# laboshinl/loam_velodyne

Hardware: AMD Instinct MI355X
Metric: sweeps/sec (64-ring, 1M-pt map): feature extraction + odometry + scan-to-map registration (higher is better)
Workload: dtype f32

## Files before the change

### loam_velodyne_amd/csrc/dev_math.hpp

```cpp
#pragma once
#include <hip/hip_runtime.h>
#include <cfloat>

namespace loamx {

struct Pose {
  float rx, ry, rz, tx, ty, tz;
  float srx, crx, sry, cry, srz, crz;
};

__host__ __device__ inline void pose_set_angles(Pose& p, float rx, float ry, float rz) {
  p.rx = rx; p.ry = ry; p.rz = rz;
  p.srx = (float)sin((double)rx); p.crx = (float)cos((double)rx);
  p.sry = (float)sin((double)ry); p.cry = (float)cos((double)ry);
  p.srz = (float)sin((double)rz); p.crz = (float)cos((double)rz);
}

__host__ __device__ inline void rot_x(float& y, float& z, float c, float s) {
  float y0 = y;
  y = c * y0 - s * z;
  z = s * y0 + c * z;
}
__host__ __device__ inline void rot_y(float& x, float& z, float c, float s) {
  float x0 = x;
// ... 332 lines not shown
__device__ __forceinline__ bool degeneracy_projector(const float* AtA, float thr, float* P, float* ws) {
  if (certainly_not_degenerate(AtA, thr)) return false;
  return degeneracy_projector_full(AtA, thr, P, ws);
}
__device__ __forceinline__ bool degeneracy_projector_full(const float* AtA, float thr, float* P, float* ws) {
  float w[6];
  float* V = ws + 72;
  float* V2 = ws + 108;
  float* Vi = ws + 144;
  eig6_sym(AtA, w, V, ws);
  for (int k = 0; k < 36; k++) V2[k] = V[k];
  bool degenerate = false;
  {
    bool go = true;
#pragma unroll
    for (int i = 0; i < 6; i++) {
      if (go && w[i] < thr) {
        for (int j = 0; j < 6; j++) V2[i * 6 + j] = 0.f;
        degenerate = true;
      } else {
        go = false;
      }
    }
  }
  if (!inverse6(V, Vi, ws)) {
    for (int k = 0; k < 36; k++) P[k] = (k % 7 == 0) ? 1.f : 0.f;
    return degenerate;
  }
  for (int r = 0; r < 6; r++)
    for (int c = 0; c < 6; c++) {
      float s = 0.f;
      for (int k = 0; k < 6; k++) s += Vi[r * 6 + k] * V2[k * 6 + c];
      P[r * 6 + c] = s;
    }
  return degenerate;
}

__device__ __forceinline__ float lane_get(float x, int lane) { return __int_as_float(__builtin_amdgcn_readlane(__float_as_int(x), lane)); }

__device__ __forceinline__ float qr_solve6_lanes(const float* AtA, const float* AtB) {
  const int gl = (int)(threadIdx.x & 63);
  float a[6];
#pragma unroll
  for (int r = 0; r < 6; r++) a[r] = gl < 6 ? AtA[r * 6 + gl] : (gl == 6 ? AtB[r] : 0.f);
  int L[6] = {0, 1, 2, 3, 4, 5};
  bool pivoted = false;
  float s0 = 0.f;
#pragma unroll
  for (int r = 0; r < 6; r++) s0 += a[r] * a[r];
  const float nrm = gl < 6 ? sqrtf(s0) : 0.f;
  float maxnorm = lane_get(nrm, 0);
#pragma unroll
  for (int c = 1; c < 6; c++) {
    const float v = lane_get(nrm, c);
    maxnorm = v > maxnorm ? v : maxnorm;
  }
  const float thr_helper = (maxnorm * FLT_EPSILON) * (maxnorm * FLT_EPSILON) / 6.0f;
  int nonzero = 6;
#pragma unroll
  for (int k = 0; k < 6; k++) {
    float s = 0.f, tail = 0.f;
#pragma unroll
    for (int r = k; r < 6; r++) s += a[r] * a[r];
#pragma unroll
    for (int r = k + 1; r < 6; r++) tail += a[r] * a[r];
    const float c0 = a[k];
    float tau, beta, v[6];
    if (tail <= FLT_MIN) {
      tau = 0.f;
      beta = c0;
#pragma unroll
      for (int r = 0; r < 6; r++) v[r] = 0.f;
    } else {
      beta = sqrtf(c0 * c0 + tail);
      if (c0 >= 0.f) beta = -beta;
#pragma unroll
      for (int r = 0; r < 6; r++) v[r] = r > k ? a[r] / (c0 - beta) : 0.f;
      tau = (beta - c0) / beta;
    }
    v[k] = 1.f;
    int best = k;
    float bestn = lane_get(s, L[k]);
#pragma unroll
    for (int c = k + 1; c < 6; c++) {
      const float sc = lane_get(s, L[c]);
      if (sc > bestn) { bestn = sc; best = c; }
    }
    best = __builtin_amdgcn_readfirstlane(best);
    if (nonzero == 6 && bestn < thr_helper * float(6 - k)) nonzero = k;
    {
      int lb = L[k];
#pragma unroll
      for (int c = k + 1; c < 6; c++) lb = best == c ? L[c] : lb;
#pragma unroll
      for (int c = k + 1; c < 6; c++) L[c] = best == c ? L[k] : L[c];
      L[k] = __builtin_amdgcn_readfirstlane(lb);
    }
    const int pl = L[k];
    tau = lane_get(tau, pl);
    beta = lane_get(beta, pl);
#pragma unroll
    for (int r = k + 1; r < 6; r++) v[r] = lane_get(v[r], pl);
    if (gl == pl) {
      pivoted = true;
      a[k] = beta;
#pragma unroll
      for (int r = k + 1; r < 6; r++) a[r] = 0.f;
    } else if (gl <= 6 && !pivoted) {
      float dot = 0.f;
#pragma unroll
      for (int r = k; r < 6; r++) dot += v[r] * a[r];
      dot *= tau;
#pragma unroll
      for (int r = k; r < 6; r++) a[r] -= dot * v[r];
    }
  }
  float y = 0.f;
#pragma unroll
  for (int k = 5; k >= 0; k--) {
    float sacc = lane_get(a[k], 6);
#pragma unroll
    for (int c = k + 1; c < 6; c++) {
      const float term = lane_get(a[k] * y, L[c]);
      if (c < nonzero) sacc -= term;
    }
    const float diag = lane_get(a[k], L[k]);
    if (gl == L[k] && k < nonzero) y = sacc / diag;
  }
  return gl < 6 ? y : 0.f;
}
__device__ __forceinline__ void qr_solve6_coop(const float* AtA, const float* AtB, float* X) {
  const float y = qr_solve6_lanes(AtA, AtB);
  if ((threadIdx.x & 63) < 6) X[threadIdx.x & 63] = y;
}

__device__ __forceinline__ void xchg_store(double* p, double v) { __hip_atomic_store(p, v, __ATOMIC_RELAXED, __HIP_MEMORY_SCOPE_AGENT); }
__device__ __forceinline__ void xchg_stores_done() { asm volatile("s_waitcnt vmcnt(0)" ::: "memory"); }
__device__ __forceinline__ double xchg_load_nowait(const double* p) {
  double v;
  asm volatile("global_load_dwordx2 %0, %1, off sc1" : "=v"(v) : "v"(p) : "memory");
  return v;
}
typedef unsigned xrec_t __attribute__((ext_vector_type(4)));
__device__ __forceinline__ void xrec_store(xrec_t* p, double v, unsigned tag) {
  xrec_t r;
  r.x = tag; r.y = (unsigned)__double2loint(v); r.z = (unsigned)__double2hiint(v); r.w = tag;
  asm volatile("global_store_dwordx4 %0, %1, off sc1\n\ts_nop 1" ::"v"(p), "v"(r) : "memory");
}
__device__ __forceinline__ xrec_t xrec_load(const xrec_t* p) {
  xrec_t r;
  asm volatile("global_load_dwordx4 %0, %1, off sc1\n\ts_waitcnt vmcnt(0)" : "=v"(r) : "v"(p) : "memory");
  return r;
}
__device__ __forceinline__ double xrec_value(const xrec_t& r) { return __hiloint2double((int)r.z, (int)r.y); }
__device__ __forceinline__ void xchg_loads_done() { asm volatile("s_waitcnt vmcnt(0)" ::: "memory"); }
__device__ __forceinline__ void xchg_loaded(double& v) { asm volatile("" : "+v"(v)); }

}
```

### loam_velodyne_amd/csrc/odometry.hip

```cpp
#include "odometry.hpp"
#include "odom_schedule.hpp"
#include "pinned_copy.hpp"
#include <chrono>
#include <cstring>
#include <type_traits>

namespace loamx {

constexpr int OD_THREADS = 256;
constexpr int OD_TR_STRIDE = OD_THREADS + 2;
constexpr int OD_PART_STRIDE = 2 * (2 * 16 * LX_NSUM) + 16;
[[maybe_unused]] constexpr int OD_PART_TS = 2 * (2 * 16 * LX_NSUM);

__device__ inline void sincos_f(float a, float& s, float& c) { sincosf(a, &s, &c); }

__device__ inline void transform_to_start(const float* T, float scan_period, const float4 pi, float& x, float& y, float& z) {
  const float s = (1.f / scan_period) * (pi.w - (float)(int)pi.w);
  x = pi.x - s * T[3];
  y = pi.y - s * T[4];
  z = pi.z - s * T[5];
  float sx, cx, sy, cy, sz, cz;
  sincos_f(-s * T[0], sx, cx);
  sincos_f(-s * T[1], sy, cy);
  sincos_f(-s * T[2], sz, cz);
  rot_z(x, y, cz, sz);
  rot_x(y, z, cx, sx);
  rot_y(x, z, cy, sy);
}

constexpr uint32_t OD_IDX_MASK = 0xffffffu;

__device__ inline float sqd(const float4& a, float x, float y, float z) {
  const float dx = a.x - x, dy = a.y - y, dz = a.z - z;
  return dx * dx + dy * dy + dz * dz;
}

__device__ inline void wave_argmin(float& d, int& j, int& order) {
#pragma unroll
  for (int off = 32; off > 0; off >>= 1) {
    const float od = __shfl_xor(d, off, 64);
    const int oj = __shfl_xor(j, off, 64);
    const int oo = __shfl_xor(order, off, 64);
    if (od < d || (od == d && oo < order)) { d = od; j = oj; order = oo; }
  }
}

__device__ inline int nn1_shells(const GridDesc& g, const float4* __restrict__ sorted, const uint32_t* __restrict__ cell_start, float qx,
                                 float qy, float qz, int lane, int L0, float best, int best_id) {
  float lbest = best;
  uint32_t lid = best_id >= 0 ? (uint32_t)best_id : 0xffffffffu;
  const float h = 1.0f / g.inv_h;
  const float fx = (qx - g.ox) * g.inv_h, fy = (qy - g.oy) * g.inv_h, fz = (qz - g.oz) * g.inv_h;
  const int cx = (int)floorf(fx), cy = (int)floorf(fy), cz = (int)floorf(fz);
  for (int L = L0;; L++) {
    const int side = 2 * L + 1, nrows = side * side;
    for (int r0 = 0; r0 < nrows; r0 += 64) {
      uint32_t b0 = 0, e0 = 0, b1 = 0, e1 = 0;
      {
        const int rr = r0 + lane;
        if (rr < nrows) {
          const int dz = rr / side - L, dy = rr % side - L;
          const int z = cz + dz, y = cy + dy;
          if (z >= 0 && z < g.nz && y >= 0 && y < g.ny) {
            const float gz = dz == 0 ? 0.f : (dz > 0 ? ((float)z - fz) : (fz - (float)(z + 1))) * h;
            const float gy = dy == 0 ? 0.f : (dy > 0 ? ((float)y - fy) : (fy - (float)(y + 1))) * h;
            const float gyz = (gy * gy + gz * gz) * 0.9999f;
            if (gyz < best) {
              const float rx = sqrtf(best - gyz) * g.inv_h * 1.0001f + 1e-3f;
              const int xlo = (int)floorf(fx - rx), xhi = (int)floorf(fx + rx);
              const bool face = (dz == -L || dz == L || dy == -L || dy == L);
              const uint32_t row = ((uint32_t)z * g.ny + y) * g.nx;
              int xa = cx - L, xb = face ? cx + L : cx - L;
              if (xa < xlo) xa = xlo;
              if (xb > xhi) xb = xhi;
              if (xa < 0) xa = 0;
              if (xb > g.nx - 1) xb = g.nx - 1;
              if (xa <= xb) { b0 = cell_start[row + xa]; e0 = cell_start[row + xb + 1]; }
              if (!face && L > 0) {
                const int xc = cx + L;
                if (xc >= xlo && xc <= xhi && xc >= 0 && xc <= g.nx - 1) { b1 = cell_start[row + xc]; e1 = cell_start[row + xc + 1]; }
              }
            }
          }
        }
      }
      unsigned long long todo = __ballot(e0 > b0 || e1 > b1);
      while (todo) {
        const int src = __builtin_ctzll(todo);
        todo &= todo - 1;
        const uint32_t rb0 = __shfl(b0, src, 64), re0 = __shfl(e0, src, 64), rb1 = __shfl(b1, src, 64), re1 = __shfl(e1, src, 64);
        for (int part = 0; part < 2; part++) {
          const uint32_t beg = part ? rb1 : rb0, end = part ? re1 : re0;
          for (uint32_t k = beg + lane; k < end; k += 64) {
            const float4 p = sorted[k];
            const float dx = qx - p.x, dy2 = qy - p.y, dz2 = qz - p.z;
            const float d2 = dx * dx + dy2 * dy2 + dz2 * dz2;
            const uint32_t id = __float_as_uint(p.w) & OD_IDX_MASK;
            if (d2 < lbest || (d2 == lbest && lid != 0xffffffffu && id < lid)) { lbest = d2; lid = id; }
          }
        }
      }
    }
    float d = lbest;
    int j = (int)lid, o_ = (int)lid;
    if (lid == 0xffffffffu) { j = -1; o_ = 0x7fffffff; }
    wave_argmin(d, j, o_);
    if (j >= 0 && d < 25.0f) { best = d; best_id = j; }
    const float cover = (float)L * h;
    if (best <= cover * cover) break;
    if (cover * cover >= 25.0f) break;
  }
  return best_id;
}
#ifdef OD_CORR_WAVES
#define OD_CORR_ATTR __attribute__((amdgpu_waves_per_eu(OD_CORR_WAVES, OD_CORR_WAVES)))
#else
#define OD_CORR_ATTR
#endif
struct Block27 {
  uint32_t E[9], O[9];
  uint32_t total;
};
__device__ inline void block27_build(const GridDesc& g, const uint32_t* __restrict__ cell_start, float qx, float qy, float qz, int lane, Block27& B) {
  const float fx = (qx - g.ox) * g.inv_h, fy = (qy - g.oy) * g.inv_h, fz = (qz - g.oz) * g.inv_h;
  const int cx = (int)floorf(fx), cy = (int)floorf(fy), cz = (int)floorf(fz);
  uint32_t v = 0u;
  {
    const int r = lane >> 1, z = cz + r / 3 - 1, y = cy + r % 3 - 1;
    if (lane < 18 && z >= 0 && z < g.nz && y >= 0 && y < g.ny) {
      int xx = (lane & 1) ? cx + 2 : cx - 1;
      xx = xx < 0 ? 0 : (xx > g.nx ? g.nx : xx);
      v = cell_start[((uint32_t)z * g.ny + y) * g.nx + xx];
    }
  }
  uint32_t acc = 0;
#pragma unroll
  for (int r = 0; r < 9; r++) {
    const uint32_t b = (uint32_t)__shfl((int)v, 2 * r, 64), e = (uint32_t)__shfl((int)v, 2 * r + 1, 64);
    B.O[r] = b - acc;
    acc += e > b ? e - b : 0u;
    B.E[r] = acc;
  }
  B.total = acc;
}
#ifndef OD_BLK_CACHE
#define OD_BLK_CACHE 2
#endif
struct Block27First { float4 p[OD_BLK_CACHE > 0 ? OD_BLK_CACHE : 1]; };
template <bool LOAD_FIRST, class F>
__device__ inline void block27_scan(const Block27& B, const float4* __restrict__ sorted, int lane, Block27First& first, F&& visit) {
  for (uint32_t c0 = (uint32_t)lane; c0 < B.total; c0 += 4 * 64) {
    const bool first_trip = c0 == (uint32_t)lane;
    uint32_t pos[4];
    float4 p[4];
#pragma unroll
    for (int u = 0; u < 4; u++) {
      const uint32_t cc = c0 + 64u * u;
      uint32_t o = B.O[8];
#pragma unroll
      for (int k = 7; k >= 0; k--) o = cc < B.E[k] ? B.O[k] : o;
      pos[u] = cc < B.total ? cc + o : B.O[0];
    }
    if (LOAD_FIRST || !first_trip) {
#pragma unroll
      for (int u = 0; u < 4; u++) p[u] = sorted[pos[u]];
      if (LOAD_FIRST && first_trip) {
#pragma unroll
        for (int u = 0; u < OD_BLK_CACHE; u++) first.p[u] = p[u];
      }
    } else {
#pragma unroll
      for (int u = OD_BLK_CACHE; u < 4; u++) p[u] = sorted[pos[u]];
#pragma unroll
      for (int u = 0; u < OD_BLK_CACHE; u++) p[u] = first.p[u];
    }
#pragma unroll
    for (int u = 0; u < 4; u++) visit(p[u], (c0 + 64u * u) < B.total);
  }
}
__device__ inline int nn1_block(const GridDesc& g, const Block27& B, const float4* __restrict__ sorted, const uint32_t* __restrict__ cell_start,
// ... 77 lines not shown
  OC_TS(3);
  if (closest < 0) {
    if (lane == 0) { pb.ind[5 * f] = -1; pb.ind[5 * f + 1] = -1; pb.ind[5 * f + 2] = -1; }
    return;
  }
  const float4* last = corner ? pb.last_corner : pb.last_surf;
  const int nLast = corner ? (int)pb.n_last_corner : (int)pb.n_last_surf;
  const int nCur = corner ? nSharp : nFlat;
  const int bound = nCur < nLast ? nCur : nLast;
  const int cscan = (wbest >> 24) != 255u ? (int)(wbest >> 24) : (int)last[closest].w;
  float d2 = 25.f, d3 = 25.f;
  int j2 = -1, j3 = -1, o2 = 0x7fffffff, o3 = 0x7fffffff;
  auto better = [](float d, int order, float dbest, int obest) { return d < dbest || (d == dbest && obest != 0x7fffffff && order < obest); };

  bool via_block = false;
  if (tbl && unordered_epoch != pb.rf_epoch && cscan < 255 && B.total > 0u) {
    const unsigned long long valid = __ballot(e0 + lane < OD_RF_N - 1 && (tv >> 24) == pb.rf_epoch);
    auto first_from = [&](int ring) -> int {
      const int k = ring - e0;
      if (k >= 64) return nLast;
      const unsigned long long m = k <= 0 ? valid : (valid >> k) << k;
      if (!m) return nLast;
      const int w = (int)((uint32_t)__shfl((int)tv, __builtin_ctzll(m), 64) & OD_IDX_MASK);
      return w < nLast ? w : nLast;
    };
    if (cscan - 2 >= e0 || e0 == 0) {
      const int wlo = min(first_from(cscan - 2), closest);
      const int whi = closest + 1 < bound ? max(min(bound, first_from(cscan + 3)), closest + 1) : closest + 1;
      const unsigned walk = (unsigned)(closest - wlo) + (unsigned)(whi - (closest + 1));
      via_block = walk > B.total + 128u;
    }
  }
  OC_TS(4);
  if (via_block) {
    block27_scan<false>(B, sorted, lane, first, [&](const float4& p, bool ok) {
      const uint32_t w = __float_as_uint(p.w);
      const int j = (int)(w & OD_IDX_MASK), ring = (int)(w >> 24);
      const float d = sqd(p, x, y, z);
      if (ok && j > closest && j < bound && ring <= cscan + 2) {
        const int order = j - (closest + 1);
        if (corner) {
          if (ring > cscan && better(d, order, d2, o2)) { d2 = d; j2 = j; o2 = order; }
        } else {
          if (ring <= cscan) { if (better(d, order, d2, o2)) { d2 = d; j2 = j; o2 = order; } }
          else { if (better(d, order, d3, o3)) { d3 = d; j3 = j; o3 = order; } }
        }
      } else if (ok && j < closest && ring >= cscan - 2) {
        const int order = 0x40000000 + (closest - 1 - j);
        if (corner) {
          if (ring < cscan && better(d, order, d2, o2)) { d2 = d; j2 = j; o2 = order; }
        } else {
          if (ring >= cscan) { if (better(d, order, d2, o2)) { d2 = d; j2 = j; o2 = order; } }
          else { if (better(d, order, d3, o3)) { d3 = d; j3 = j; o3 = order; } }
        }
      }
    });
    wave_argmin(d2, j2, o2);
    if (!corner) wave_argmin(d3, j3, o3);
    const float h = 1.0f / gd.g.inv_h, h2 = h * h;
    via_block = d2 < h2 && (corner || d3 < h2);
    if (!via_block) { d2 = d3 = 25.f; j2 = j3 = -1; o2 = o3 = 0x7fffffff; }
  }
  OC_TS(5);
  if (!via_block) {
    int baseF = closest + 1, baseB = closest - 1;
    bool stopF = baseF >= bound, stopB = baseB < 0;
    while (!stopF || !stopB) {
      float4 qf[4], qb[4];
      if (!stopF) {
#pragma unroll
        for (int u = 0; u < 4; u++) {
          const int j = baseF + 64 * u + lane;
          qf[u] = j < bound ? last[j] : make_float4(0.f, 0.f, 0.f, 0.f);
        }
      }
      if (!stopB) {
#pragma unroll
        for (int u = 0; u < 4; u++) {
          const int j = baseB - 64 * u - lane;
          qb[u] = j >= 0 ? last[j] : make_float4(0.f, 0.f, 0.f, 0.f);
        }
      }
      if (!stopF) {
        bool stop = false;
#pragma unroll
        for (int u = 0; u < 4; u++) {
          if (stop) continue;
          const int j = baseF + 64 * u + lane;
          const bool in = j < bound;
          const int ring = (int)qf[u].w;
          const bool brk = in && ((double)ring > (double)cscan + 2.5);
          const unsigned long long mb = __ballot(brk);
          const int fb = mb ? __builtin_ctzll(mb) : 64;
          if (in && lane < fb) {
            const float d = sqd(qf[u], x, y, z);
            const int order = j - (closest + 1);
            if (corner) {
              if (ring > cscan && better(d, order, d2, o2)) { d2 = d; j2 = j; o2 = order; }
            } else {
              if (ring <= cscan) { if (better(d, order, d2, o2)) { d2 = d; j2 = j; o2 = order; } }
              else { if (better(d, order, d3, o3)) { d3 = d; j3 = j; o3 = order; } }
            }
          }
          if (mb) stop = true;
        }
        baseF += 256;
        stopF = stop || baseF >= bound;
      }
      if (!stopB) {
        bool stop = false;
#pragma unroll
        for (int u = 0; u < 4; u++) {
          if (stop) continue;
          const int j = baseB - 64 * u - lane;
          const bool in = j >= 0;
          const int ring = (int)qb[u].w;
          const bool brk = in && ((double)ring < (double)cscan - 2.5);
          const unsigned long long mb = __ballot(brk);
          const int fb = mb ? __builtin_ctzll(mb) : 64;
          if (in && lane < fb) {
            const float d = sqd(qb[u], x, y, z);
            const int order = 0x40000000 + (closest - 1 - j);
            if (corner) {
              if (ring < cscan && better(d, order, d2, o2)) { d2 = d; j2 = j; o2 = order; }
            } else {
              if (ring >= cscan) { if (better(d, order, d2, o2)) { d2 = d; j2 = j; o2 = order; } }
              else { if (better(d, order, d3, o3)) { d3 = d; j3 = j; o3 = order; } }
            }
          }
          if (mb) stop = true;
        }
        baseB -= 256;
        stopB = stop || baseB < 0;
      }
    }
    wave_argmin(d2, j2, o2);
    if (!corner) wave_argmin(d3, j3, o3);
  }
  OC_TS(6);
  if (lane == 0) {
    pb.ind[5 * f] = closest;
    pb.ind[5 * f + 1] = j2;
    pb.ind[5 * f + 2] = corner ? -1 : j3;
  }
#ifdef LOAMX_PROF_CORR
  if (blockIdx.y == 0 && lane == 0 && ts_slot >= 0) {
    g_corr_ts[ts_slot][7] = wall_clock64();
    g_corr_ts[ts_slot][8] = (unsigned long long)B.total; g_corr_ts[ts_slot][9] = (unsigned long long)via_block;
    g_corr_ts[ts_slot][10] = (unsigned long long)closest; g_corr_ts[ts_slot][11] = (unsigned long long)cscan;
  }
#endif
}

#ifdef LOAMX_PROF_LM
#define LM_TS(k) do { if (blockIdx.x == 0 && blockIdx.y == 0 && tid == 0 && iter == it_begin + 1) pb.part[OD_PART_TS + (k)] = (double)wall_clock64(); } while (0)
#else
#define LM_TS(k) do { } while (0)
#endif
#ifndef OD_LM_WAVES
#define OD_LM_WAVES 3
#endif
#ifndef OD_LM_WAVES_MIN
#define OD_LM_WAVES_MIN 3
#endif
#define OD_LM_ATTR __attribute__((amdgpu_waves_per_eu(OD_LM_WAVES_MIN, OD_LM_WAVES)))
#pragma clang diagnostic push
#pragma clang diagnostic ignored "-Wpass-failed"
template <int OD_FPT>
__global__ __launch_bounds__(OD_THREADS) OD_LM_ATTR void k_odom_lm(OdomProblem* __restrict__ probs, OdomParams P, int iter0, int n_iters) {
  OdomProblem& pb = probs[blockIdx.y];
  if (pb.done) return;
  const unsigned NB = gridDim.x;
  const int tid = threadIdx.x;
  const int nSharp = (int)pb.n_sharp, nFlat = (int)pb.n_flat, nFeat = nSharp + nFlat;
  __shared__ float T[6];
  __shared__ float trig[6];
  __shared__ double red[8][LX_NSUM];
  using TrT = typename std::conditional<OD_FPT == 1, float, double>::type;
  __shared__ TrT tr[LX_NSUM * OD_TR_STRIDE];
  __shared__ int sh_done, sh_degen, sh_abort;
  __shared__ float matP[36];
  __shared__ float ws[216];
  __shared__ double parts[16 * LX_NSUM];
  __shared__ float AtA[36], AtB[6];
  if (tid < 6) {
    T[tid] = pb.transform[tid];
    const double ang = (double)pb.transform[tid >> 1];
    trig[tid] = (float)((tid & 1) ? cos(ang) : sin(ang));
  }
  const unsigned xtag = pb.xchg_epoch << 8;
  if (tid == 0) { sh_done = 0; sh_abort = 0; sh_degen = pb.stats.degenerate; }
  if (tid < 36) matP[tid] = pb.matP[tid];
  __syncthreads();

  float4 fpo[OD_FPT], ft1[OD_FPT], ft2[OD_FPT], ft3[OD_FPT];
  bool fvalid[OD_FPT], fcorner[OD_FPT];
#pragma unroll
  for (int u = 0; u < OD_FPT; u++) {
    const int f = (u * (int)NB + (int)blockIdx.x) * OD_THREADS + tid;
    fvalid[u] = false;
    fcorner[u] = f < nSharp;
    fpo[u] = ft1[u] = ft2[u] = ft3[u] = make_float4(0.f, 0.f, 0.f, 0.f);
    if (f < nFeat) {
      const int i1 = pb.ind[5 * f], i2 = pb.ind[5 * f + 1], i3 = pb.ind[5 * f + 2];
      if (fcorner[u] ? (i2 >= 0) : (i2 >= 0 && i3 >= 0)) {
        fvalid[u] = true;
        fpo[u] = fcorner[u] ? pb.sharp[f] : pb.flat[f - nSharp];
        const float4* last = fcorner[u] ? pb.last_corner : pb.last_surf;
        ft1[u] = last[i1];
        ft2[u] = last[i2];
        if (!fcorner[u]) ft3[u] = last[i3];
      }
    }
  }

  const int it_begin = iter0, it_end = iter0 + n_iters;
  for (int iter = it_begin; iter < it_end; iter++) {
    LM_TS(0);
    LM_TS(1);
    double v[OD_FPT == 1 ? 1 : LX_NSUM];
    float a1[6] = {0.f, 0.f, 0.f, 0.f, 0.f, 0.f}, bb1 = 0.f;
    bool sel1 = false;
#pragma unroll
    for (int k = 0; k < (OD_FPT == 1 ? 1 : LX_NSUM); k++) v[k] = 0.0;
#pragma unroll
    for (int u = 0; u < OD_FPT; u++) {
      if (!fvalid[u]) continue;
      const bool corner = fcorner[u];
      const float4 po = fpo[u];
      float cx = 0.f, cy = 0.f, cz = 0.f, ci = 0.f;
      bool sel = false;
      {
        float x0, y0, z0;
        transform_to_start(T, P.scan_period, po, x0, y0, z0);
        if (corner) {
          const float4 t1 = ft1[u], t2 = ft2[u];
          const float x1 = t1.x, y1 = t1.y, z1 = t1.z, x2 = t2.x, y2 = t2.y, z2 = t2.z;
          const float a012 = sqrtf(((x0 - x1) * (y0 - y2) - (x0 - x2) * (y0 - y1)) * ((x0 - x1) * (y0 - y2) - (x0 - x2) * (y0 - y1)) +
                                   ((x0 - x1) * (z0 - z2) - (x0 - x2) * (z0 - z1)) * ((x0 - x1) * (z0 - z2) - (x0 - x2) * (z0 - z1)) +
                                   ((y0 - y1) * (z0 - z2) - (y0 - y2) * (z0 - z1)) * ((y0 - y1) * (z0 - z2) - (y0 - y2) * (z0 - z1)));
          const float l12 = sqrtf((x1 - x2) * (x1 - x2) + (y1 - y2) * (y1 - y2) + (z1 - z2) * (z1 - z2));
          const float la = ((y1 - y2) * ((x0 - x1) * (y0 - y2) - (x0 - x2) * (y0 - y1)) +
                            (z1 - z2) * ((x0 - x1) * (z0 - z2) - (x0 - x2) * (z0 - z1))) / a012 / l12;
          const float lb = -((x1 - x2) * ((x0 - x1) * (y0 - y2) - (x0 - x2) * (y0 - y1)) -
                             (z1 - z2) * ((y0 - y1) * (z0 - z2) - (y0 - y2) * (z0 - z1))) / a012 / l12;
          const float lc = -((x1 - x2) * ((x0 - x1) * (z0 - z2) - (x0 - x2) * (z0 - z1)) +
                             (y1 - y2) * ((y0 - y1) * (z0 - z2) - (y0 - y2) * (z0 - z1))) / a012 / l12;
          const float ld2 = a012 / l12;
          float s = 1;
          if (iter >= 5) s = 1 - 1.8f * fabsf(ld2);
          cx = s * la; cy = s * lb; cz = s * lc; ci = s * ld2;
          sel = ((double)s > 0.1) && (ld2 != 0);
        } else {
          const float4 t1 = ft1[u], t2 = ft2[u], t3 = ft3[u];
          float pa = (t2.y - t1.y) * (t3.z - t1.z) - (t3.y - t1.y) * (t2.z - t1.z);
          float pbb = (t2.z - t1.z) * (t3.x - t1.x) - (t3.z - t1.z) * (t2.x - t1.x);
          float pc = (t2.x - t1.x) * (t3.y - t1.y) - (t3.x - t1.x) * (t2.y - t1.y);
          float pd = -(pa * t1.x + pbb * t1.y + pc * t1.z);
          const float ps = sqrtf(pa * pa + pbb * pbb + pc * pc);
          pa /= ps; pbb /= ps; pc /= ps; pd /= ps;
          const float pd2 = pa * x0 + pbb * y0 + pc * z0 + pd;
          float s = 1;
          if (iter >= 5) s = 1 - 1.8f * fabsf(pd2) / sqrtf(sqrtf(x0 * x0 + y0 * y0 + z0 * z0));
          cx = s * pa; cy = s * pbb; cz = s * pc; ci = s * pd2;
          sel = ((double)s > 0.1) && (pd2 != 0);
        }
      }
      if (sel) {
        const float srx = trig[0], crx = trig[1], sry = trig[2], cry = trig[3], srz = trig[4], crz = trig[5];
        const float tx = T[3], ty = T[4], tz = T[5];
        const float px = po.x, py = po.y, pz = po.z;
        float a[6];
        a[0] = (-crx * sry * srz * px + crx * crz * sry * py + srx * sry * pz + tx * crx * sry * srz - ty * crx * crz * sry - tz * srx * sry) * cx +
               (srx * srz * px - crz * srx * py + crx * pz + ty * crz * srx - tz * crx - tx * srx * srz) * cy +
               (crx * cry * srz * px - crx * cry * crz * py - cry * srx * pz + tz * cry * srx + ty * crx * cry * crz - tx * crx * cry * srz) * cz;
        a[1] = ((-crz * sry - cry * srx * srz) * px + (cry * crz * srx - sry * srz) * py - crx * cry * pz + tx * (crz * sry + cry * srx * srz) +
                ty * (sry * srz - cry * crz * srx) + tz * crx * cry) * cx +
               ((cry * crz - srx * sry * srz) * px + (cry * srz + crz * srx * sry) * py - crx * sry * pz + tz * crx * sry -
                ty * (cry * srz + crz * srx * sry) - tx * (cry * crz - srx * sry * srz)) * cz;
        a[2] = ((-cry * srz - crz * srx * sry) * px + (cry * crz - srx * sry * srz) * py + tx * (cry * srz + crz * srx * sry) -
                ty * (cry * crz - srx * sry * srz)) * cx +
               (-crx * crz * px - crx * srz * py + ty * crx * srz + tx * crx * crz) * cy +
               ((cry * crz * srx - sry * srz) * px + (crz * sry + cry * srx * srz) * py + tx * (sry * srz - cry * crz * srx) -
                ty * (crz * sry + cry * srx * srz)) * cz;
        a[3] = -(cry * crz - srx * sry * srz) * cx + crx * srz * cy - (crz * sry + cry * srx * srz) * cz;
        a[4] = -(cry * srz + crz * srx * sry) * cx - crx * crz * cy - (sry * srz - cry * crz * srx) * cz;
        a[5] = crx * sry * cx - srx * cy - crx * cry * cz;
        const float bb = (float)(-0.05 * (double)ci);
        if (OD_FPT == 1) {
#pragma unroll
          for (int i = 0; i < 6; i++) a1[i] = a[i];
          bb1 = bb;
          sel1 = true;
        } else {
          int k = 0;
#pragma unroll
          for (int i = 0; i < 6; i++)
#pragma unroll
            for (int j = i; j < 6; j++) v[k++] += (double)(a[i] * a[j]);
#pragma unroll
          for (int i = 0; i < 6; i++) v[k++] += (double)(a[i] * bb);
          v[k] += 1.0;
        }
      }
    }
    LM_TS(2);
    if (OD_FPT == 1) {
      int k = 0;
#pragma unroll
      for (int i = 0; i < 6; i++)
#pragma unroll
        for (int j = i; j < 6; j++) tr[(k++) * OD_TR_STRIDE + tid] = (TrT)(a1[i] * a1[j]);
#pragma unroll
      for (int i = 0; i < 6; i++) tr[(k++) * OD_TR_STRIDE + tid] = (TrT)(a1[i] * bb1);
      tr[k * OD_TR_STRIDE + tid] = (TrT)(sel1 ? 1.f : 0.f);
    } else {
#pragma unroll
      for (int t = 0; t < LX_NSUM; t++) tr[t * OD_TR_STRIDE + tid] = (TrT)v[OD_FPT == 1 ? 0 : t];
    }
    __syncthreads();
    if (tid < 8 * LX_NSUM) {
      const int c = tid % LX_NSUM, g = tid / LX_NSUM;
      const TrT* col = tr + c * OD_TR_STRIDE + g;
      double x = 0.0;
#pragma unroll 8
      for (int j = 0; j < OD_THREADS / 8; j++) x += (double)col[8 * j];
      red[g][c] = x;
    }
    __syncthreads();
    LM_TS(3);
    double xs = 0.0;
    if (tid < LX_NSUM) {
#pragma unroll
      for (int w = 0; w < 8; w++) xs += red[w][tid];
      if (NB > 1) {
        xrec_store(reinterpret_cast<xrec_t*>(pb.part) + (((unsigned)iter & 1u) * 16u + blockIdx.x) * LX_NSUM + tid, xs, xtag | (unsigned)(iter + 1));
      }
    }
    if (NB > 1) {
      LM_TS(4);
      {
        const unsigned want = xtag | (unsigned)(iter + 1);
        const xrec_t* rec = reinterpret_cast<const xrec_t*>(pb.part) + ((unsigned)iter & 1u) * 16u * LX_NSUM;
        const unsigned long long t_in = wall_clock64();
        for (unsigned e = tid; e < NB * LX_NSUM; e += OD_THREADS) {
          unsigned spins = 0;
          xrec_t r = xrec_load(rec + e);
          while (r.x != want || r.w != want) {
            __builtin_amdgcn_s_sleep(1);
            if ((++spins & 1023u) == 0u && wall_clock64() - t_in > 200000000ull) { sh_abort = 1; break; }
            r = xrec_load(rec + e);
          }
          parts[e] = xrec_value(r);
        }
      }
      __syncthreads();
      if (sh_abort) {
        if (tid == 0) {
          pb.done = 1;
          if (pb.err_word) __hip_atomic_store(pb.err_word, 1u, __ATOMIC_RELAXED, __HIP_MEMORY_SCOPE_SYSTEM);
          if (pb.host_mirror) pb.host_mirror->done = -1;
        }
        return;
      }
      LM_TS(5);
    }
    if (tid < 64) {
      if (NB > 1 && tid < LX_NSUM) {
        xs = 0.0;
        for (unsigned b = 0; b < NB; b++) xs += parts[b * LX_NSUM + tid];
      }
      if (tid < 21) {
        int i = 0, rem = tid;
        while (rem >= 6 - i) { rem -= 6 - i; i++; }
        const int j = i + rem;
        AtA[i * 6 + j] = AtA[j * 6 + i] = (float)xs;
      } else if (tid < 27) {
        AtB[tid - 21] = (float)xs;
      }
      const int sel = (int)__hiloint2double(__builtin_amdgcn_readlane(__double2hiint(xs), 27), __builtin_amdgcn_readlane(__double2loint(xs), 27));
      __builtin_amdgcn_fence(__ATOMIC_SEQ_CST, "wavefront");
      LM_TS(7);
      float xl = 0.f;
      int done_now = 0;
      if (sel >= 10) {
        xl = qr_solve6_lanes(AtA, AtB);
        LM_TS(8);
        if (iter == 0) {
          if (tid == 0) sh_degen = degeneracy_projector(AtA, 10.f, matP, ws) ? 1 : 0;
          __builtin_amdgcn_fence(__ATOMIC_SEQ_CST, "wavefront");
          if (blockIdx.x == 0 && tid < 36) pb.matP[tid] = matP[tid];
        }
        const int degen = sh_degen;
        if (degen) {
          const int r = tid < 6 ? tid : 5;
          float acc = 0.f;
#pragma unroll
          for (int c = 0; c < 6; c++) acc += matP[r * 6 + c] * lane_get(xl, c);
          xl = acc;
        }
        float x6[6];
#pragma unroll
        for (int k = 0; k < 6; k++) x6[k] = lane_get(xl, k);
        const float d0 = (float)(x6[0] * 180.0 / M_PI), d1 = (float)(x6[1] * 180.0 / M_PI), d2 = (float)(x6[2] * 180.0 / M_PI);
        const float deltaR = (float)sqrt((double)d0 * d0 + (double)d1 * d1 + (double)d2 * d2);
        const float t0 = x6[3] * 100, t1 = x6[4] * 100, t2 = x6[5] * 100;
        const float deltaT = (float)sqrt((double)t0 * t0 + (double)t1 * t1 + (double)t2 * t2);
        done_now = (deltaR < P.delta_r_abort && deltaT < P.delta_t_abort) ? 1 : 0;
      }
      float tl = T[tid < 6 ? tid : 5];
      if (sel >= 10) {
        float nv = tl + xl;
        if (!isfinite(nv)) nv = 0.f;
        tl = nv;
      }
      const float a0 = lane_get(tl, 0), a1 = lane_get(tl, 1), a2 = lane_get(tl, 2);
      const double ang = (double)((tid >> 1) == 0 ? a0 : ((tid >> 1) == 1 ? a1 : a2));
      const float tg = (float)((tid & 1) ? cos(ang) : sin(ang));
      if (tid < 6) { T[tid] = tl; trig[tid] = tg; }
      if (tid == 0 && done_now) sh_done = 1;
      if (blockIdx.x == 0) {
        const bool final_now = done_now || iter == it_end - 1;
        if (tid < 6) pb.transform[tid] = tl;
        if (tid == 0) {
          pb.stats.iterations = iter + 1;
          pb.stats.sel = sel;
          if (iter == 0 && sel >= 10) pb.stats.degenerate = sh_degen;
          if (done_now) pb.done = 1;
        }
        if (final_now) {
          ToEndParams& Pe = *pb.te_out;
          if (tid < 6) {
            Pe.T[tid] = tl;
            if (tid & 1) Pe.cT[tid >> 1] = tg; else Pe.sT[tid >> 1] = tg;
          }
          if (pb.host_mirror) {
            OdomProblem* hm = pb.host_mirror;
            if (tid < 6) hm->transform[tid] = tl;
            if (tid == 0) {
              OdomStats stt;
              stt.iterations = iter + 1; stt.sel = sel; stt.frame = pb.stats.frame; stt.degenerate = sh_degen;
              hm->stats = stt;
              hm->done = done_now;
            }
          }
        }
      }
      LM_TS(9);
    }
    __syncthreads();
    if (sh_done) break;
  }
}

#pragma clang diagnostic pop

__device__ inline float4 to_end_point(float4 p, const ToEndParams& P) {
  const float s = (1.f / P.scan_period) * (p.w - (float)(int)p.w);
  float x = p.x - s * P.T[3], y = p.y - s * P.T[4], z = p.z - s * P.T[5];
  float sx, cx, sy, cy, sz, cz;
  sincos_f(-s * P.T[0], sx, cx);
  sincos_f(-s * P.T[1], sy, cy);
  sincos_f(-s * P.T[2], sz, cz);
  rot_z(x, y, cz, sz); rot_x(y, z, cx, sx); rot_y(x, z, cy, sy);
  rot_y(x, z, P.cT[1], P.sT[1]); rot_x(y, z, P.cT[0], P.sT[0]); rot_z(x, y, P.cT[2], P.sT[2]);
  x += P.T[3] - P.shift[0];
  y += P.T[4] - P.shift[1];
  z += P.T[5] - P.shift[2];
  rot_z(x, y, P.c_start[2], P.s_start[2]); rot_x(y, z, P.c_start[0], P.s_start[0]); rot_y(x, z, P.c_start[1], P.s_start[1]);
  rot_y(x, z, P.c_end[1], -P.s_end[1]); rot_x(y, z, P.c_end[0], -P.s_end[0]); rot_z(x, y, P.c_end[2], -P.s_end[2]);
  return make_float4(x, y, z, (float)(int)p.w);
}
__global__ __launch_bounds__(256) void k_transform_to_end_copy(float4* __restrict__ dst, const float4* __restrict__ src, uint32_t n, ToEndParams P) {
  const uint32_t i = blockIdx.x * blockDim.x + threadIdx.x;
  if (i >= n) return;
  dst[i] = to_end_point(src[i], P);
}
__global__ __launch_bounds__(256) void k_transform_to_end(float4* __restrict__ pts, uint32_t n, ToEndParams P) {
  const uint32_t i = blockIdx.x * blockDim.x + threadIdx.x;
  if (i >= n) return;
  pts[i] = to_end_point(pts[i], P);
}
__global__ void k_te_patch(const OdomProblem* __restrict__ probs, uint32_t na, ToEndParams* __restrict__ te) {
  const uint32_t a = blockIdx.x * blockDim.x + threadIdx.x;
  if (a >= na) return;
  const OdomProblem& pb = probs[a];
  ToEndParams& P = te[pb.stream_id];
  for (int k = 0; k < 6; k++) P.T[k] = pb.transform[k];
  for (int k = 0; k < 3; k++) {
    P.sT[k] = (float)sin((double)pb.transform[k]);
    P.cT[k] = (float)cos((double)pb.transform[k]);
  }
}

__global__ __launch_bounds__(256) void k_transform_to_end_batch(float4* __restrict__ pts, uint32_t n, const uint32_t* __restrict__ off,
                                                                uint32_t K, uint32_t ns, const ToEndParams* __restrict__ params,
                                                                const float4* __restrict__ src_c, const float4* __restrict__ src_s,
                                                                uint32_t n_corner_all, uint32_t* __restrict__ bounds,
                                                                uint32_t* __restrict__ ring_first, uint32_t rf_epoch) {
  const uint32_t i = blockIdx.x * blockDim.x + threadIdx.x;
  const bool active = i < n;
  uint32_t lo = 0;
  float4 q = make_float4(0.f, 0.f, 0.f, 0.f);
  if (active) {
    uint32_t hi = K;
    while (hi - lo > 1) {
      const uint32_t mid = (lo + hi) >> 1;
      if (off[mid] <= i) lo = mid; else hi = mid;
    }
    const ToEndParams P = params[lo % ns];
    if (src_c) {
      const float4 p = i < n_corner_all ? src_c[i] : src_s[i - n_corner_all];
      q = P.enabled ? to_end_point(p, P) : p;
      pts[i] = q;
    } else {
      q = pts[i];
      if (P.enabled) { q = to_end_point(q, P); pts[i] = q; }
    }
  }
  if (ring_first) {
    const int ring = (int)q.w;
    int prev = __shfl_up(ring, 1, 64);
    const uint32_t plo = (uint32_t)__shfl_up((int)lo, 1, 64);
    const bool first_in_cloud = active && i == off[lo];
    if (active && !first_in_cloud && (threadIdx.x & 63) == 0) {
      const uint32_t ip = i - 1;
      prev = (int)(src_c ? (ip < n_corner_all ? src_c[ip] : src_s[ip - n_corner_all]) : pts[ip]).w;
    } else if (active && plo != lo) {
      prev = -1;
    }
    if (active && ring >= 0 && ring < OD_RF_N - 1 && (first_in_cloud || prev != ring))
      ring_first[(size_t)lo * OD_RF_N + ring] = (rf_epoch << 24) | ((i - off[lo]) & OD_IDX_MASK);
    if (active && (ring < 0 || ring >= 255 || (i - off[lo]) > OD_IDX_MASK || (!first_in_cloud && prev > ring)))
      ring_first[(size_t)lo * OD_RF_N + OD_RF_N - 1] = rf_epoch;
  }
  if (bounds) cloud_bounds_update(bounds, active, lo, q.x, q.y, q.z);
}

__global__ __launch_bounds__(256) void k_to_end_gather(float4* __restrict__ dst, uint32_t n, const uint32_t* __restrict__ off, uint32_t K,
                                                       const float4* const* __restrict__ src, const uint32_t* __restrict__ sid,
                                                       const ToEndParams* __restrict__ params) {
  const uint32_t i = blockIdx.x * blockDim.x + threadIdx.x;
  if (i >= n) return;
  uint32_t lo = 0, hi = K;
  while (hi - lo > 1) {
    const uint32_t mid = (lo + hi) >> 1;
    if (off[mid] <= i) lo = mid; else hi = mid;
  }
  dst[i] = to_end_point(src[lo][i - off[lo]], params[sid[lo]]);
}

OdometryBatch::OdometryBatch(int device, uint32_t n_streams, hipStream_t shared_stream) : device_(device) {
  select_device(device);
  LX_REQUIRE(n_streams >= 1 && n_streams <= 1024, "n_streams must be in [1, 1024]");
  if (shared_stream) {
    st_ = shared_stream;
  } else {
    st_ = create_stream(env_priority("LOAMX_PRIO_ODOM", +1), 0, 0);
    own_stream_ = true;
  }
  for (uint32_t s = 0; s < n_streams; s++) streams_.push_back(new OdomStream());
  index_.cell_size = 2.1f;
  if (const char* e = diag_env("LOAMX_ODOM_CELL")) { const float v = (float)atof(e); if (v >= 0.25f && v <= 16.f) index_.cell_size = v; }
  index_.pack_ring = true;
  index_.init(st_);
  h_mirror_.reserve(n_streams);
  h_err_.reserve(16);
  rf_.reserve((size_t)2 * n_streams * OD_RF_N);
  LX_HIP(hipMemsetAsync(rf_.p, 0, sizeof(uint32_t) * 2 * n_streams * OD_RF_N, st_));
  memset(h_err_.p, 0, 16 * sizeof(uint32_t));
  part_.reserve((size_t)n_streams * OD_PART_STRIDE);
  LX_HIP(hipMemset(part_.p, 0, sizeof(double) * part_.cap));
  {
    auto up256 = [](size_t b) { return (b + 255) & ~(size_t)255; };
    const size_t o_te = up256(sizeof(OdomProblem) * n_streams), o_off = o_te + up256(sizeof(ToEndParams) * n_streams);
    up_bytes_ = o_off + up256(sizeof(uint32_t) * (2 * (size_t)n_streams + 2));
    up_dev_.reserve(up_bytes_);
    up_host_.reserve(up_bytes_);
    memset(up_host_.p, 0, up_bytes_);
    prob_.p = (OdomProblem*)up_dev_.p; h_prob_.p = (OdomProblem*)up_host_.p;
    te_.p = (ToEndParams*)(up_dev_.p + o_te); h_te_.p = (ToEndParams*)(up_host_.p + o_te);
    d_cur_off_.p = (uint32_t*)(up_dev_.p + o_off); h_off_pin_.p = (uint32_t*)(up_host_.p + o_off);
  }
  h_cur_off_.assign(2 * n_streams + 1, 0);
  h_last_off_.assign(2 * n_streams + 1, 0);
}

OdometryBatch::~OdometryBatch() {
  if (ev_tail_) (void)hipEventDestroy(ev_tail_);
  if (ev_up_) (void)hipEventDestroy(ev_up_);
  if (ev_pose_) (void)hipEventDestroy(ev_pose_);
  for (auto* p : streams_) delete p;
  for (auto& c : lt_) for (auto& e : c.ev) if (e) (void)hipEventDestroy(e);
  if (own_stream_ && st_) (void)hipStreamDestroy(st_);
}

void OdometryBatch::lt_resolve_() {
  for (auto& c : lt_) {
    if (!c.pending || !c.pairs) continue;
    if (hipEventQuery(c.ev[3 * (c.pairs - 1) + 2]) != hipSuccess) { (void)hipGetLastError(); continue; }
    for (int k = 0; k < c.pairs; k++) {
      float a = 0.f, b = 0.f;
      if (hipEventElapsedTime(&a, c.ev[3 * k], c.ev[3 * k + 1]) != hipSuccess || hipEventElapsedTime(&b, c.ev[3 * k + 1], c.ev[3 * k + 2]) != hipSuccess) { (void)hipGetLastError(); continue; }
// ... 528 lines not shown
```

Baseline: 15420.

## Precompute per-feature LM geometry and poll cross-block partials from a single wave

Loop-invariant per-feature data (sweep fraction, corner line endpoints and length, surface plane coefficients) is now computed once before the LM iteration loop instead of every iteration. The cross-block partial-sum exchange is now polled by wave 0 alone, with four batched loads per poll and a wave-wide any() check. This drops one block-wide __syncthreads from each iteration, and the abort handling moves to after the existing end-of-iteration barrier. It trades register pressure from the cached LmFeat structs for less per-iteration ALU work and shorter synchronisation latency.

```diff
diff --git a/loam_velodyne_amd/csrc/dev_math.hpp b/loam_velodyne_amd/csrc/dev_math.hpp
--- a/loam_velodyne_amd/csrc/dev_math.hpp
+++ b/loam_velodyne_amd/csrc/dev_math.hpp
@@ -508,6 +508,14 @@
   asm volatile("global_load_dwordx4 %0, %1, off sc1\n\ts_waitcnt vmcnt(0)" : "=v"(r) : "v"(p) : "memory");
   return r;
 }
+__device__ __forceinline__ void xrec_load4(const xrec_t* p0, const xrec_t* p1, const xrec_t* p2, const xrec_t* p3, xrec_t (&r)[4]) {
+  asm volatile(
+      "global_load_dwordx4 %0, %4, off sc1\n\tglobal_load_dwordx4 %1, %5, off sc1\n\tglobal_load_dwordx4 %2, %6, off sc1\n\t"
+      "global_load_dwordx4 %3, %7, off sc1\n\ts_waitcnt vmcnt(0)"
+      : "=&v"(r[0]), "=&v"(r[1]), "=&v"(r[2]), "=&v"(r[3])
+      : "v"(p0), "v"(p1), "v"(p2), "v"(p3)
+      : "memory");
+}
 __device__ __forceinline__ double xrec_value(const xrec_t& r) { return __hiloint2double((int)r.z, (int)r.y); }
 __device__ __forceinline__ void xchg_loads_done() { asm volatile("s_waitcnt vmcnt(0)" ::: "memory"); }
 __device__ __forceinline__ void xchg_loaded(double& v) { asm volatile("" : "+v"(v)); }
diff --git a/loam_velodyne_amd/csrc/odometry.hip b/loam_velodyne_amd/csrc/odometry.hip
--- a/loam_velodyne_amd/csrc/odometry.hip
+++ b/loam_velodyne_amd/csrc/odometry.hip
@@ -14,11 +14,11 @@
 
 __device__ inline void sincos_f(float a, float& s, float& c) { sincosf(a, &s, &c); }
 
-__device__ inline void transform_to_start(const float* T, float scan_period, const float4 pi, float& x, float& y, float& z) {
-  const float s = (1.f / scan_period) * (pi.w - (float)(int)pi.w);
-  x = pi.x - s * T[3];
-  y = pi.y - s * T[4];
-  z = pi.z - s * T[5];
+__device__ inline float sweep_fraction(float scan_period, const float4 pi) { return (1.f / scan_period) * (pi.w - (float)(int)pi.w); }
+__device__ inline void transform_to_start_s(const float* T, float s, float px, float py, float pz, float& x, float& y, float& z) {
+  x = px - s * T[3];
+  y = py - s * T[4];
+  z = pz - s * T[5];
   float sx, cx, sy, cy, sz, cz;
   sincos_f(-s * T[0], sx, cx);
   sincos_f(-s * T[1], sy, cy);
@@ -26,6 +26,9 @@
   rot_z(x, y, cz, sz);
   rot_x(y, z, cx, sx);
   rot_y(x, z, cy, sy);
+}
+__device__ inline void transform_to_start(const float* T, float scan_period, const float4 pi, float& x, float& y, float& z) {
+  transform_to_start_s(T, sweep_fraction(scan_period, pi), pi.x, pi.y, pi.z, x, y, z);
 }
 
 constexpr uint32_t OD_IDX_MASK = 0xffffffu;
@@ -409,6 +412,32 @@
 #endif
 }
 
+
+struct LmFeat {
+  float px, py, pz;
+  float s;
+  float g[7];
+};
+__device__ inline LmFeat lm_feat(bool corner, const float4 po, const float4 t1, const float4 t2, const float4 t3, float scan_period) {
+  LmFeat e;
+  e.px = po.x; e.py = po.y; e.pz = po.z;
+  e.s = sweep_fraction(scan_period, po);
+  if (corner) {
+    const float x1 = t1.x, y1 = t1.y, z1 = t1.z, x2 = t2.x, y2 = t2.y, z2 = t2.z;
+    e.g[0] = x1; e.g[1] = y1; e.g[2] = z1; e.g[3] = x2; e.g[4] = y2; e.g[5] = z2;
+    e.g[6] = sqrtf((x1 - x2) * (x1 - x2) + (y1 - y2) * (y1 - y2) + (z1 - z2) * (z1 - z2));
+  } else {
+    float pa = (t2.y - t1.y) * (t3.z - t1.z) - (t3.y - t1.y) * (t2.z - t1.z);
+    float pbb = (t2.z - t1.z) * (t3.x - t1.x) - (t3.z - t1.z) * (t2.x - t1.x);
+    float pc = (t2.x - t1.x) * (t3.y - t1.y) - (t3.x - t1.x) * (t2.y - t1.y);
+    float pd = -(pa * t1.x + pbb * t1.y + pc * t1.z);
+    const float ps = sqrtf(pa * pa + pbb * pbb + pc * pc);
+    pa /= ps; pbb /= ps; pc /= ps; pd /= ps;
+    e.g[0] = pa; e.g[1] = pbb; e.g[2] = pc; e.g[3] = pd; e.g[4] = e.g[5] = e.g[6] = 0.f;
+  }
+  return e;
+}
+
 #ifdef LOAMX_PROF_LM
 #define LM_TS(k) do { if (blockIdx.x == 0 && blockIdx.y == 0 && tid == 0 && iter == it_begin + 1) pb.part[OD_PART_TS + (k)] = (double)wall_clock64(); } while (0)
 #else
@@ -440,6 +469,20 @@
   __shared__ float ws[216];
   __shared__ double parts[16 * LX_NSUM];
   __shared__ float AtA[36], AtB[6];
+  int fi1[OD_FPT], fi2[OD_FPT], fi3[OD_FPT];
+  float4 fpo[OD_FPT];
+  bool fcorner[OD_FPT];
+#pragma unroll
+  for (int u = 0; u < OD_FPT; u++) {
+    const int f = (u * (int)NB + (int)blockIdx.x) * OD_THREADS + tid;
+    fcorner[u] = f < nSharp;
+    fi1[u] = fi2[u] = fi3[u] = -1;
+    fpo[u] = make_float4(0.f, 0.f, 0.f, 0.f);
+    if (f < nFeat) {
+      fi1[u] = pb.ind[5 * f]; fi2[u] = pb.ind[5 * f + 1]; fi3[u] = pb.ind[5 * f + 2];
+      fpo[u] = fcorner[u] ? pb.sharp[f] : pb.flat[f - nSharp];
+    }
+  }
   if (tid < 6) {
     T[tid] = pb.transform[tid];
     const double ang = (double)pb.transform[tid >> 1];
@@ -448,28 +491,21 @@
   const unsigned xtag = pb.xchg_epoch << 8;
   if (tid == 0) { sh_done = 0; sh_abort = 0; sh_degen = pb.stats.degenerate; }
   if (tid < 36) matP[tid] = pb.matP[tid];
+  LmFeat fe[OD_FPT];
+  bool fvalid[OD_FPT];
+#pragma unroll
+  for (int u = 0; u < OD_FPT; u++) {
+    fvalid[u] = fcorner[u] ? (fi2[u] >= 0) : (fi2[u] >= 0 && fi3[u] >= 0);
+    float4 t1 = make_float4(0.f, 0.f, 0.f, 0.f), t2 = t1, t3 = t1;
+    if (fvalid[u]) {
+      const float4* last = fcorner[u] ? pb.last_corner : pb.last_surf;
+      t1 = last[fi1[u]];
+      t2 = last[fi2[u]];
+      if (!fcorner[u]) t3 = last[fi3[u]];
+    }
+    fe[u] = lm_feat(fcorner[u], fpo[u], t1, t2, t3, P.scan_period);
+  }
   __syncthreads();
-
-  float4 fpo[OD_FPT], ft1[OD_FPT], ft2[OD_FPT], ft3[OD_FPT];
-  bool fvalid[OD_FPT], fcorner[OD_FPT];
-#pragma unroll
-  for (int u = 0; u < OD_FPT; u++) {
-    const int f = (u * (int)NB + (int)blockIdx.x) * OD_THREADS + tid;
-    fvalid[u] = false;
-    fcorner[u] = f < nSharp;
-    fpo[u] = ft1[u] = ft2[u] = ft3[u] = make_float4(0.f, 0.f, 0.f, 0.f);
-    if (f < nFeat) {
-      const int i1 = pb.ind[5 * f], i2 = pb.ind[5 * f + 1], i3 = pb.ind[5 * f + 2];
-      if (fcorner[u] ? (i2 >= 0) : (i2 >= 0 && i3 >= 0)) {
-        fvalid[u] = true;
-        fpo[u] = fcorner[u] ? pb.sharp[f] : pb.flat[f - nSharp];
-        const float4* last = fcorner[u] ? pb.last_corner : pb.last_surf;
-        ft1[u] = last[i1];
-        ft2[u] = last[i2];
-        if (!fcorner[u]) ft3[u] = last[i3];
-      }
-    }
-  }
 
   const int it_begin = iter0, it_end = iter0 + n_iters;
   for (int iter = it_begin; iter < it_end; iter++) {
@@ -484,19 +520,17 @@
     for (int u = 0; u < OD_FPT; u++) {
       if (!fvalid[u]) continue;
       const bool corner = fcorner[u];
-      const float4 po = fpo[u];
+      const LmFeat& e = fe[u];
       float cx = 0.f, cy = 0.f, cz = 0.f, ci = 0.f;
       bool sel = false;
       {
         float x0, y0, z0;
-        transform_to_start(T, P.scan_period, po, x0, y0, z0);
+        transform_to_start_s(T, e.s, e.px, e.py, e.pz, x0, y0, z0);
         if (corner) {
-          const float4 t1 = ft1[u], t2 = ft2[u];
-          const float x1 = t1.x, y1 = t1.y, z1 = t1.z, x2 = t2.x, y2 = t2.y, z2 = t2.z;
+          const float x1 = e.g[0], y1 = e.g[1], z1 = e.g[2], x2 = e.g[3], y2 = e.g[4], z2 = e.g[5], l12 = e.g[6];
           const float a012 = sqrtf(((x0 - x1) * (y0 - y2) - (x0 - x2) * (y0 - y1)) * ((x0 - x1) * (y0 - y2) - (x0 - x2) * (y0 - y1)) +
                                    ((x0 - x1) * (z0 - z2) - (x0 - x2) * (z0 - z1)) * ((x0 - x1) * (z0 - z2) - (x0 - x2) * (z0 - z1)) +
                                    ((y0 - y1) * (z0 - z2) - (y0 - y2) * (z0 - z1)) * ((y0 - y1) * (z0 - z2) - (y0 - y2) * (z0 - z1)));
-          const float l12 = sqrtf((x1 - x2) * (x1 - x2) + (y1 - y2) * (y1 - y2) + (z1 - z2) * (z1 - z2));
           const float la = ((y1 - y2) * ((x0 - x1) * (y0 - y2) - (x0 - x2) * (y0 - y1)) +
                             (z1 - z2) * ((x0 - x1) * (z0 - z2) - (x0 - x2) * (z0 - z1))) / a012 / l12;
           const float lb = -((x1 - x2) * ((x0 - x1) * (y0 - y2) - (x0 - x2) * (y0 - y1)) -
@@ -509,13 +543,7 @@
           cx = s * la; cy = s * lb; cz = s * lc; ci = s * ld2;
           sel = ((double)s > 0.1) && (ld2 != 0);
         } else {
-          const float4 t1 = ft1[u], t2 = ft2[u], t3 = ft3[u];
-          float pa = (t2.y - t1.y) * (t3.z - t1.z) - (t3.y - t1.y) * (t2.z - t1.z);
-          float pbb = (t2.z - t1.z) * (t3.x - t1.x) - (t3.z - t1.z) * (t2.x - t1.x);
-          float pc = (t2.x - t1.x) * (t3.y - t1.y) - (t3.x - t1.x) * (t2.y - t1.y);
-          float pd = -(pa * t1.x + pbb * t1.y + pc * t1.z);
-          const float ps = sqrtf(pa * pa + pbb * pbb + pc * pc);
-          pa /= ps; pbb /= ps; pc /= ps; pd /= ps;
+          const float pa = e.g[0], pbb = e.g[1], pc = e.g[2], pd = e.g[3];
           const float pd2 = pa * x0 + pbb * y0 + pc * z0 + pd;
           float s = 1;
           if (iter >= 5) s = 1 - 1.8f * fabsf(pd2) / sqrtf(sqrtf(x0 * x0 + y0 * y0 + z0 * z0));
@@ -526,7 +554,7 @@
       if (sel) {
         const float srx = trig[0], crx = trig[1], sry = trig[2], cry = trig[3], srz = trig[4], crz = trig[5];
         const float tx = T[3], ty = T[4], tz = T[5];
-        const float px = po.x, py = po.y, pz = po.z;
+        const float px = e.px, py = e.py, pz = e.pz;
         float a[6];
         a[0] = (-crx * sry * srz * px + crx * crz * sry * py + srx * sry * pz + tx * crx * sry * srz - ty * crx * crz * sry - tz * srx * sry) * cx +
                (srx * srz * px - crz * srx * py + crx * pz + ty * crz * srx - tz * crx - tx * srx * srz) * cy +
@@ -594,35 +622,39 @@
         xrec_store(reinterpret_cast<xrec_t*>(pb.part) + (((unsigned)iter & 1u) * 16u + blockIdx.x) * LX_NSUM + tid, xs, xtag | (unsigned)(iter + 1));
       }
     }
-    if (NB > 1) {
+    bool aborted = false;
+    if (NB > 1 && tid < 64) {
       LM_TS(4);
-      {
-        const unsigned want = xtag | (unsigned)(iter + 1);
-        const xrec_t* rec = reinterpret_cast<const xrec_t*>(pb.part) + ((unsigned)iter & 1u) * 16u * LX_NSUM;
-        const unsigned long long t_in = wall_clock64();
-        for (unsigned e = tid; e < NB * LX_NSUM; e += OD_THREADS) {
-          unsigned spins = 0;
-          xrec_t r = xrec_load(rec + e);
-          while (r.x != want || r.w != want) {
-            __builtin_amdgcn_s_sleep(1);
-            if ((++spins & 1023u) == 0u && wall_clock64() - t_in > 200000000ull) { sh_abort = 1; break; }
-            r = xrec_load(rec + e);
-          }
-          parts[e] = xrec_value(r);
-        }
-      }
-      __syncthreads();
-      if (sh_abort) {
-        if (tid == 0) {
-          pb.done = 1;
-          if (pb.err_word) __hip_atomic_store(pb.err_word, 1u, __ATOMIC_RELAXED, __HIP_MEMORY_SCOPE_SYSTEM);
-          if (pb.host_mirror) pb.host_mirror->done = -1;
-        }
-        return;
-      }
+      const unsigned want = xtag | (unsigned)(iter + 1);
+      const xrec_t* rec = reinterpret_cast<const xrec_t*>(pb.part) + ((unsigned)iter & 1u) * 16u * LX_NSUM;
+      const unsigned nrec = NB * LX_NSUM;
+      const unsigned long long t_in = wall_clock64();
+      unsigned spins = 0;
+      for (unsigned base = 0; base < nrec && !aborted; base += 256u) {
+        xrec_t r[4];
+        unsigned e[4];
+#pragma unroll
+        for (int u = 0; u < 4; u++) e[u] = base + 64u * (unsigned)u + (unsigned)tid;
+        for (;;) {
+          xrec_load4(rec + min(e[0], nrec - 1u), rec + min(e[1], nrec - 1u), rec + min(e[2], nrec - 1u), rec + min(e[3], nrec - 1u), r);
+          bool miss = false;
+#pragma unroll
+          for (int u = 0; u < 4; u++) miss |= r[u].x != want || r[u].w != want;
+          if (!__any(miss)) break;
+          __builtin_amdgcn_s_sleep(1);
+          if ((++spins & 1023u) == 0u && wall_clock64() - t_in > 200000000ull) { aborted = true; break; }
+        }
+        if (!aborted) {
+#pragma unroll
+          for (int u = 0; u < 4; u++)
+            if (e[u] < nrec) parts[e[u]] = xrec_value(r[u]);
+        }
+      }
+      if (aborted && tid == 0) sh_abort = 1;
+      __builtin_amdgcn_fence(__ATOMIC_SEQ_CST, "wavefront");
       LM_TS(5);
     }
-    if (tid < 64) {
+    if (tid < 64 && !aborted) {
       if (NB > 1 && tid < LX_NSUM) {
         xs = 0.0;
         for (unsigned b = 0; b < NB; b++) xs += parts[b * LX_NSUM + tid];
@@ -706,6 +738,14 @@
       LM_TS(9);
     }
     __syncthreads();
+    if (NB > 1 && sh_abort) {
+      if (tid == 0) {
+        pb.done = 1;
+        if (pb.err_word) __hip_atomic_store(pb.err_word, 1u, __ATOMIC_RELAXED, __HIP_MEMORY_SCOPE_SYSTEM);
+        if (pb.host_mirror) pb.host_mirror->done = -1;
+      }
+      return;
+    }
     if (sh_done) break;
   }
 }
```

After: 14820. 3.9% lower.
